# quoroom-ai/room

Measured on AMD Instinct MI355X. Metric: agent-cycles/sec, higher is better.
Workload: dtype bf16; 1 GPU; model=qwen3-coder-30b, agents_per_gpu=5, global_batch=5, seq_len=dynamic (session KV), parallelism=swarm-shard dp1 (one room shard/GPU, RCCL quorum)

## Files before the change

### room_amd/ops/csrc/flash_prefill.hip

```cpp
#include <torch/extension.h>
#include <c10/hip/HIPStream.h>
#include "common.h"
#include "kv_fp8.h"
#include "checks.h"

#define FP_BS 16
#define FP_QTOK 32
#define FP_CHUNK 64
#define FP_D 128
#define FP_QH 8
#define FP_PADK 8

typedef __attribute__((ext_vector_type(4))) float fpfrag_t;

template <bool F8>
__global__ __launch_bounds__(512, 1)
void flash_prefill_kernel(short* __restrict__ out,
                          const short* __restrict__ q,
                          const std::conditional_t<F8, uint8_t, short>*
                              __restrict__ kcache,
                          const std::conditional_t<F8, uint8_t, short>*
                              __restrict__ vcache,
                          const int* __restrict__ block_table,
                          const int* __restrict__ seq_ids,
                          const int* __restrict__ q_pos,
                          const int* __restrict__ tile_desc,
                          int n_kvheads, int max_blocks, int q_row_stride,
                          float scale,
                          const float* __restrict__ kscale,
                          const float* __restrict__ vscale) {
  const int g = blockIdx.x;
  const int hk = blockIdx.y;
  const int row0 = tile_desc[g * 2 + 0];
  const int ntok = tile_desc[g * 2 + 1];
  const int tid = threadIdx.x;
  const int wid = tid >> 6;
  const int lane = tid & 63;
  const int n_qheads = n_kvheads * FP_QH;
  const int hq = hk * FP_QH + wid;

  __shared__ short q_s[FP_QH][FP_QTOK][FP_D + FP_PADK];
  __shared__ short k_s[FP_CHUNK][FP_D + FP_PADK];
  __shared__ short vt_s[FP_D][FP_CHUNK + FP_PADK];
  __shared__ short p_s[FP_QH][FP_QTOK][FP_CHUNK + FP_PADK];
  __shared__ int qp_s[FP_QTOK];
  __shared__ int seq_s;

  #pragma unroll
  for (int it = 0; it < 8; ++it) {
    const int idx = tid + it * 512;
    const int h = idx / (FP_QTOK * FP_D / 8);
    const int rem = idx % (FP_QTOK * FP_D / 8);
    const int tk = rem / (FP_D / 8);
    const int d8 = (rem % (FP_D / 8)) * 8;
    bf16x8 v = {0, 0, 0, 0, 0, 0, 0, 0};
    if (tk < ntok) {
      v = *reinterpret_cast<const bf16x8*>(
          q + (long)(row0 + tk) * q_row_stride + (hk * FP_QH + h) * FP_D + d8);
      #pragma unroll
      for (int j = 0; j < 8; ++j) v[j] = f2bf(bf2f(v[j]) * scale);
    }
    *reinterpret_cast<bf16x8*>(&q_s[h][tk][d8]) = v;
  }
  if (tid < FP_QTOK)
    qp_s[tid] = (tid < ntok) ? q_pos[row0 + tid] : -1;
  if (tid == 0) seq_s = seq_ids[row0];
  __syncthreads();

  const int seq = seq_s;
  int bound_max = 0, bound_min = INT_MAX;
  for (int i = 0; i < ntok; ++i) {
    bound_max = max(bound_max, qp_s[i] + 1);
    bound_min = min(bound_min, qp_s[i] + 1);
  }
  const int* btab = block_table + (long)seq * max_blocks;
  const long kv_stride_block = (long)n_kvheads * FP_BS * FP_D;

  float m_run[2][4], l_run[2][4];
  fpfrag_t oacc[2][8];
  #pragma unroll
  for (int mt = 0; mt < 2; ++mt) {
    #pragma unroll
    for (int r = 0; r < 4; ++r) { m_run[mt][r] = -INFINITY; l_run[mt][r] = 0.f; }
    #pragma unroll
    for (int nf = 0; nf < 8; ++nf) oacc[mt][nf] = fpfrag_t{0.f, 0.f, 0.f, 0.f};
  }

  for (int base = 0; base < bound_max; base += FP_CHUNK) {
    #pragma unroll
    for (int it = 0; it < 2; ++it) {
      const int idx = tid + it * 512;
      const int pos_l = (idx * 8) / FP_D;
      const int d8 = (idx * 8) % FP_D;
      const int pos = base + pos_l;
      bf16x8 kv = {0, 0, 0, 0, 0, 0, 0, 0};
      bf16x8 vv = {0, 0, 0, 0, 0, 0, 0, 0};
      if (pos < bound_max) {
        const int blk = btab[pos / FP_BS];
        const long off = (long)blk * kv_stride_block
                         + ((long)hk * FP_BS + (pos % FP_BS)) * FP_D + d8;
        if constexpr (F8) {
          const long soff = ((long)blk * n_kvheads + hk) * FP_BS + pos % FP_BS;
          const kv_u32x2 kq = *reinterpret_cast<const kv_u32x2*>(kcache + off);
          const kv_u32x2 vq = *reinterpret_cast<const kv_u32x2*>(vcache + off);
          kv = __builtin_bit_cast(bf16x8, kv_fp8x8_to_bf16(kq, kscale[soff]));
          vv = __builtin_bit_cast(bf16x8, kv_fp8x8_to_bf16(vq, vscale[soff]));
        } else {
          kv = *reinterpret_cast<const bf16x8*>(kcache + off);
          vv = *reinterpret_cast<const bf16x8*>(vcache + off);
        }
      }
      *reinterpret_cast<bf16x8*>(&k_s[pos_l][d8]) = kv;
      #pragma unroll
      for (int j = 0; j < 8; ++j) vt_s[d8 + j][pos_l] = vv[j];
    }
    __syncthreads();

    fpfrag_t sfrag[2][4];
    #pragma unroll
    for (int mt = 0; mt < 2; ++mt)
      #pragma unroll
      for (int nt = 0; nt < 4; ++nt)
        sfrag[mt][nt] = fpfrag_t{0.f, 0.f, 0.f, 0.f};
    #pragma unroll
    for (int kk = 0; kk < 4; ++kk) {
      const int akoff = kk * 32 + (lane >> 4) * 8;
      bf16x8 a0 = *reinterpret_cast<const bf16x8*>(&q_s[wid][lane & 15][akoff]);
      bf16x8 a1 = *reinterpret_cast<const bf16x8*>(
          &q_s[wid][16 + (lane & 15)][akoff]);
      #pragma unroll
      for (int nt = 0; nt < 4; ++nt) {
        bf16x8 b = *reinterpret_cast<const bf16x8*>(
            &k_s[nt * 16 + (lane & 15)][akoff]);
        sfrag[0][nt] = __builtin_amdgcn_mfma_f32_16x16x32_bf16(a0, b, sfrag[0][nt], 0, 0, 0);
        sfrag[1][nt] = __builtin_amdgcn_mfma_f32_16x16x32_bf16(a1, b, sfrag[1][nt], 0, 0, 0);
      }
    }

    const int colL = lane & 15;
    const bool interior = (ntok == FP_QTOK) && (base + FP_CHUNK <= bound_min);
    #pragma unroll
    for (int mt = 0; mt < 2; ++mt) {
      #pragma unroll
      for (int r = 0; r < 4; ++r) {
        const int tk = mt * 16 + (lane >> 4) * 4 + r;
        const int bound = qp_s[tk] + 1;
        float sv[4];
        float mx = -INFINITY;
        if (interior) {
          #pragma unroll
          for (int nt = 0; nt < 4; ++nt) {
            sv[nt] = sfrag[mt][nt][r];
            mx = fmaxf(mx, sv[nt]);
          }
        } else {
          #pragma unroll
          for (int nt = 0; nt < 4; ++nt) {
            float s = sfrag[mt][nt][r];
            if (base + nt * 16 + colL >= bound) s = -INFINITY;
            sv[nt] = s;
            mx = fmaxf(mx, s);
          }
        }
        #pragma unroll
        for (int off = 8; off > 0; off >>= 1)
          mx = fmaxf(mx, __shfl_xor(mx, off, WAVE));
        const float m_new = fmaxf(m_run[mt][r], mx);
        float rs = 1.f, lsum = 0.f;
        float pv[4] = {0.f, 0.f, 0.f, 0.f};
        if (m_new != -INFINITY) {
          rs = (m_run[mt][r] == -INFINITY) ? 1.f : __expf(m_run[mt][r] - m_new);
          #pragma unroll
          for (int nt = 0; nt < 4; ++nt) {
            pv[nt] = (sv[nt] == -INFINITY) ? 0.f : __expf(sv[nt] - m_new);
            lsum += pv[nt];
          }
          #pragma unroll
          for (int off = 8; off > 0; off >>= 1)
            lsum += __shfl_xor(lsum, off, WAVE);
          l_run[mt][r] = l_run[mt][r] * rs + lsum;
          m_run[mt][r] = m_new;
        }
        #pragma unroll
        for (int nt = 0; nt < 4; ++nt)
          p_s[wid][tk][nt * 16 + colL] = f2bf(pv[nt]);
        if (rs != 1.f) {
          #pragma unroll
          for (int nf = 0; nf < 8; ++nf) oacc[mt][nf][r] *= rs;
        }
      }
    }
    __syncthreads();

    #pragma unroll
    for (int kk = 0; kk < 2; ++kk) {
      const int akoff = kk * 32 + (lane >> 4) * 8;
      bf16x8 a0 = *reinterpret_cast<const bf16x8*>(&p_s[wid][lane & 15][akoff]);
      bf16x8 a1 = *reinterpret_cast<const bf16x8*>(
          &p_s[wid][16 + (lane & 15)][akoff]);
      #pragma unroll
      for (int nf = 0; nf < 8; ++nf) {
        bf16x8 b = *reinterpret_cast<const bf16x8*>(
            &vt_s[nf * 16 + (lane & 15)][akoff]);
        oacc[0][nf] = __builtin_amdgcn_mfma_f32_16x16x32_bf16(a0, b, oacc[0][nf], 0, 0, 0);
        oacc[1][nf] = __builtin_amdgcn_mfma_f32_16x16x32_bf16(a1, b, oacc[1][nf], 0, 0, 0);
      }
    }
    __syncthreads();
  }

  #pragma unroll
  for (int mt = 0; mt < 2; ++mt) {
    #pragma unroll
    for (int r = 0; r < 4; ++r) {
      const int tk = mt * 16 + (lane >> 4) * 4 + r;
      if (tk >= ntok) continue;
      const float inv_l = (l_run[mt][r] > 0.f) ? 1.0f / l_run[mt][r] : 0.f;
      #pragma unroll
      for (int nf = 0; nf < 8; ++nf) {
        out[((long)(row0 + tk) * n_qheads + hq) * FP_D + nf * 16 + (lane & 15)] =
            f2bf(oacc[mt][nf][r] * inv_l);
      }
    }
  }
}

void flash_prefill(torch::Tensor out, torch::Tensor q, torch::Tensor kcache,
                   torch::Tensor vcache, torch::Tensor block_table,
                   torch::Tensor seq_ids, torch::Tensor q_pos,
                   torch::Tensor tile_desc, double scale,
                   c10::optional<torch::Tensor> k_scale,
                   c10::optional<torch::Tensor> v_scale) {
  OpChecks c("flash_prefill");
  const bool fp8 = kv_fp8_check(c, kcache, vcache, k_scale, v_scale);
  attn_check_tokens(c, out, q, kcache, block_table, seq_ids, q_pos);
  c.tensor("tile_desc", tile_desc, kI32, {-1, 2});
  const int n_kvheads = kcache.size(1);
  const int G = c.fits_int("tile_desc.size(0)", tile_desc.size(0));
  c.grid(G, n_kvheads);
  if (check_only()) return;
  const int max_blocks = block_table.size(1);
  dim3 grid(G, n_kvheads), block(512);
  hipStream_t s = c10::hip::getCurrentHIPStream();
  if (fp8)
    hipLaunchKernelGGL(flash_prefill_kernel<true>, grid, block, 0, s,
                       (short*)out.data_ptr(), (const short*)q.data_ptr(),
                       (const uint8_t*)kcache.data_ptr(),
                       (const uint8_t*)vcache.data_ptr(),
                       block_table.data_ptr<int>(), seq_ids.data_ptr<int>(),
                       q_pos.data_ptr<int>(), tile_desc.data_ptr<int>(),
                       n_kvheads, max_blocks, (int)q.stride(0), (float)scale,
                       k_scale->data_ptr<float>(), v_scale->data_ptr<float>());
  else
    hipLaunchKernelGGL(flash_prefill_kernel<false>, grid, block, 0, s,
                       (short*)out.data_ptr(), (const short*)q.data_ptr(),
                       (const short*)kcache.data_ptr(),
                       (const short*)vcache.data_ptr(),
                       block_table.data_ptr<int>(), seq_ids.data_ptr<int>(),
                       q_pos.data_ptr<int>(), tile_desc.data_ptr<int>(),
                       n_kvheads, max_blocks, (int)q.stride(0), (float)scale,
                       (const float*)nullptr, (const float*)nullptr);
  HIP_CHECK_KERNEL();
}

int64_t flash_prefill_qtile() { return FP_QTOK; }
```

Baseline: 6.390 cycles/s.

## Restructure flash prefill: register Q, double-buffered swizzled KV LDS, transposed V reads

Keeps Q fragments in registers instead of LDS and computes S transposed (K as the A operand), so the softmax probabilities stay in registers and feed the PV MFMA directly without a P round-trip through LDS. K/V tiles are double-buffered in XOR-swizzled LDS, and the next chunk's global loads are issued before the current chunk's compute, leaving one barrier per iteration. V is read with ds_read_tr16 transposed loads instead of a scalar transpose on store, and outputs are written packed. This adds register pressure and swizzle/transpose index complexity in exchange for less LDS traffic, fewer bank conflicts, fewer syncs and overlap of global loads with compute.

```diff
diff --git a/room_amd/ops/csrc/flash_prefill.hip b/room_amd/ops/csrc/flash_prefill.hip
--- a/room_amd/ops/csrc/flash_prefill.hip
+++ b/room_amd/ops/csrc/flash_prefill.hip
@@ -9,9 +9,17 @@
 #define FP_CHUNK 64
 #define FP_D 128
 #define FP_QH 8
-#define FP_PADK 8
+#define FP_TILE_B (FP_CHUNK * FP_D * 2)
 
 typedef __attribute__((ext_vector_type(4))) float fpfrag_t;
+typedef __attribute__((ext_vector_type(2))) float fp_f32x2;
+typedef __attribute__((ext_vector_type(2))) __bf16 fp_bf16x2;
+typedef __attribute__((address_space(3))) bf16x4 fp_lds_bf16x4;
+
+DEV uint32_t fp_pack_bf16(float lo, float hi) {
+  return __builtin_bit_cast(
+      uint32_t, __builtin_convertvector(fp_f32x2{lo, hi}, fp_bf16x2));
+}
 
 template <bool F8>
 __global__ __launch_bounds__(512, 1)
@@ -33,194 +41,237 @@
   const int hk = blockIdx.y;
   const int row0 = tile_desc[g * 2 + 0];
   const int ntok = tile_desc[g * 2 + 1];
+  if (ntok <= 0) return;
   const int tid = threadIdx.x;
   const int wid = tid >> 6;
   const int lane = tid & 63;
+  const int lrow = lane & 15;
+  const int lgrp = lane >> 4;
   const int n_qheads = n_kvheads * FP_QH;
   const int hq = hk * FP_QH + wid;
 
-  __shared__ short q_s[FP_QH][FP_QTOK][FP_D + FP_PADK];
-  __shared__ short k_s[FP_CHUNK][FP_D + FP_PADK];
-  __shared__ short vt_s[FP_D][FP_CHUNK + FP_PADK];
-  __shared__ short p_s[FP_QH][FP_QTOK][FP_CHUNK + FP_PADK];
-  __shared__ int qp_s[FP_QTOK];
-  __shared__ int seq_s;
-
-  #pragma unroll
-  for (int it = 0; it < 8; ++it) {
-    const int idx = tid + it * 512;
-    const int h = idx / (FP_QTOK * FP_D / 8);
-    const int rem = idx % (FP_QTOK * FP_D / 8);
-    const int tk = rem / (FP_D / 8);
-    const int d8 = (rem % (FP_D / 8)) * 8;
-    bf16x8 v = {0, 0, 0, 0, 0, 0, 0, 0};
+  __shared__ __attribute__((aligned(16))) char kv_s[2][2][FP_TILE_B];
+
+  bf16x8 qf[2][4];
+  int bnd[2];
+  #pragma unroll
+  for (int mt = 0; mt < 2; ++mt) {
+    const int tk = mt * 16 + lrow;
+    bnd[mt] = 0;
+    #pragma unroll
+    for (int kk = 0; kk < 4; ++kk) qf[mt][kk] = bf16x8{0, 0, 0, 0, 0, 0, 0, 0};
     if (tk < ntok) {
-      v = *reinterpret_cast<const bf16x8*>(
-          q + (long)(row0 + tk) * q_row_stride + (hk * FP_QH + h) * FP_D + d8);
-      #pragma unroll
-      for (int j = 0; j < 8; ++j) v[j] = f2bf(bf2f(v[j]) * scale);
-    }
-    *reinterpret_cast<bf16x8*>(&q_s[h][tk][d8]) = v;
+      bnd[mt] = q_pos[row0 + tk] + 1;
+      const short* qp = q + (long)(row0 + tk) * q_row_stride + hq * FP_D
+                        + lgrp * 8;
+      #pragma unroll
+      for (int kk = 0; kk < 4; ++kk) {
+        bf16x8 v = *reinterpret_cast<const bf16x8*>(qp + kk * 32);
+        #pragma unroll
+        for (int j = 0; j < 8; ++j) v[j] = f2bf(bf2f(v[j]) * scale);
+        qf[mt][kk] = v;
+      }
+    }
   }
-  if (tid < FP_QTOK)
-    qp_s[tid] = (tid < ntok) ? q_pos[row0 + tid] : -1;
-  if (tid == 0) seq_s = seq_ids[row0];
-  __syncthreads();
-
-  const int seq = seq_s;
-  int bound_max = 0, bound_min = INT_MAX;
-  for (int i = 0; i < ntok; ++i) {
-    bound_max = max(bound_max, qp_s[i] + 1);
-    bound_min = min(bound_min, qp_s[i] + 1);
+  int bmax = max(bnd[0], bnd[1]), bmin = min(bnd[0], bnd[1]);
+  #pragma unroll
+  for (int off = 8; off > 0; off >>= 1) {
+    bmax = max(bmax, __shfl_xor(bmax, off, WAVE));
+    bmin = min(bmin, __shfl_xor(bmin, off, WAVE));
   }
+  const int bound_max = __builtin_amdgcn_readfirstlane(bmax);
+  const int bound_min = __builtin_amdgcn_readfirstlane(bmin);
+
+  const int seq = seq_ids[row0];
   const int* btab = block_table + (long)seq * max_blocks;
   const long kv_stride_block = (long)n_kvheads * FP_BS * FP_D;
 
-  float m_run[2][4], l_run[2][4];
+  using raw_t = std::conditional_t<F8, kv_u32x2, bf16x8>;
+  const int srow = tid >> 4, sch = tid & 15;
+  const long slice_off = ((long)hk * FP_BS + (srow & 15)) * FP_D + sch * 8;
+  const int k_wr = srow * 256 + ((sch ^ (srow & 15)) << 4);
+  const int v_wr = srow * 256 + ((sch ^ ((srow & 7) << 1)) << 4);
+  raw_t kraw[2], vraw[2];
+  float ksc[2], vsc[2];
+  int blk[2];
+
+  auto load_blk = [&](int base) {
+    #pragma unroll
+    for (int it = 0; it < 2; ++it) {
+      const int pos = base + srow + it * 32;
+      blk[it] = (pos < bound_max) ? btab[pos / FP_BS] : 0;
+    }
+  };
+  auto issue = [&](int base) {
+    #pragma unroll
+    for (int it = 0; it < 2; ++it) {
+      const int pos = base + srow + it * 32;
+      kraw[it] = raw_t{};
+      vraw[it] = raw_t{};
+      ksc[it] = vsc[it] = 1.f;
+      if (pos < bound_max) {
+        const long off = (long)blk[it] * kv_stride_block + slice_off;
+        kraw[it] = *reinterpret_cast<const raw_t*>(kcache + off);
+        vraw[it] = *reinterpret_cast<const raw_t*>(vcache + off);
+        if constexpr (F8) {
+          const long soff = ((long)blk[it] * n_kvheads + hk) * FP_BS
+                            + (srow & 15);
+          ksc[it] = kscale[soff];
+          vsc[it] = vscale[soff];
+        }
+      }
+    }
+  };
+  auto commit = [&](int b) {
+    #pragma unroll
+    for (int it = 0; it < 2; ++it) {
+      bf16x8 kv, vv;
+      if constexpr (F8) {
+        kv = __builtin_bit_cast(bf16x8, kv_fp8x8_to_bf16(kraw[it], ksc[it]));
+        vv = __builtin_bit_cast(bf16x8, kv_fp8x8_to_bf16(vraw[it], vsc[it]));
+      } else {
+        kv = kraw[it];
+        vv = vraw[it];
+      }
+      *reinterpret_cast<bf16x8*>(&kv_s[b][0][k_wr + it * 32 * 256]) = kv;
+      *reinterpret_cast<bf16x8*>(&kv_s[b][1][v_wr + it * 32 * 256]) = vv;
+    }
+  };
+
+  int k_rd[4];
+  #pragma unroll
+  for (int kk = 0; kk < 4; ++kk)
+    k_rd[kk] = lrow * 256 + (((kk * 4 + lgrp) ^ lrow) << 4);
+  const int v_q = lrow >> 2, v_p = lrow & 3;
+  const int v_x = 4 * (lgrp & 1) + v_q;
+  const int v_rd = (4 * lgrp + v_q) * 256 + v_p * 8;
+
+  float m_run[2] = {-INFINITY, -INFINITY};
+  float l_run[2] = {0.f, 0.f};
   fpfrag_t oacc[2][8];
   #pragma unroll
-  for (int mt = 0; mt < 2; ++mt) {
-    #pragma unroll
-    for (int r = 0; r < 4; ++r) { m_run[mt][r] = -INFINITY; l_run[mt][r] = 0.f; }
+  for (int mt = 0; mt < 2; ++mt)
     #pragma unroll
     for (int nf = 0; nf < 8; ++nf) oacc[mt][nf] = fpfrag_t{0.f, 0.f, 0.f, 0.f};
-  }
-
-  for (int base = 0; base < bound_max; base += FP_CHUNK) {
-    #pragma unroll
-    for (int it = 0; it < 2; ++it) {
-      const int idx = tid + it * 512;
-      const int pos_l = (idx * 8) / FP_D;
-      const int d8 = (idx * 8) % FP_D;
-      const int pos = base + pos_l;
-      bf16x8 kv = {0, 0, 0, 0, 0, 0, 0, 0};
-      bf16x8 vv = {0, 0, 0, 0, 0, 0, 0, 0};
-      if (pos < bound_max) {
-        const int blk = btab[pos / FP_BS];
-        const long off = (long)blk * kv_stride_block
-                         + ((long)hk * FP_BS + (pos % FP_BS)) * FP_D + d8;
-        if constexpr (F8) {
-          const long soff = ((long)blk * n_kvheads + hk) * FP_BS + pos % FP_BS;
-          const kv_u32x2 kq = *reinterpret_cast<const kv_u32x2*>(kcache + off);
-          const kv_u32x2 vq = *reinterpret_cast<const kv_u32x2*>(vcache + off);
-          kv = __builtin_bit_cast(bf16x8, kv_fp8x8_to_bf16(kq, kscale[soff]));
-          vv = __builtin_bit_cast(bf16x8, kv_fp8x8_to_bf16(vq, vscale[soff]));
-        } else {
-          kv = *reinterpret_cast<const bf16x8*>(kcache + off);
-          vv = *reinterpret_cast<const bf16x8*>(vcache + off);
+
+  load_blk(0);
+  issue(0);
+  load_blk(FP_CHUNK);
+  commit(0);
+  __syncthreads();
+
+  int cur = 0;
+  for (int base = 0; base < bound_max; base += FP_CHUNK, cur ^= 1) {
+    const bool more = base + FP_CHUNK < bound_max;
+    if (more) {
+      issue(base + FP_CHUNK);
+      load_blk(base + 2 * FP_CHUNK);
+    }
+    const char* kb = kv_s[cur][0];
+    const char* vb = kv_s[cur][1];
+
+    fpfrag_t st[2][4];
+    #pragma unroll
+    for (int mt = 0; mt < 2; ++mt)
+      #pragma unroll
+      for (int nt = 0; nt < 4; ++nt)
+        st[mt][nt] = fpfrag_t{0.f, 0.f, 0.f, 0.f};
+    #pragma unroll
+    for (int kk = 0; kk < 4; ++kk) {
+      #pragma unroll
+      for (int nt = 0; nt < 4; ++nt) {
+        const bf16x8 a = *reinterpret_cast<const bf16x8*>(
+            kb + nt * 16 * 256 + k_rd[kk]);
+        st[0][nt] = __builtin_amdgcn_mfma_f32_16x16x32_bf16(a, qf[0][kk], st[0][nt], 0, 0, 0);
+        st[1][nt] = __builtin_amdgcn_mfma_f32_16x16x32_bf16(a, qf[1][kk], st[1][nt], 0, 0, 0);
+      }
+    }
+
+    const bool interior = (ntok == FP_QTOK) && (base + FP_CHUNK <= bound_min);
+    float rs[2];
+    bf16x8 pb[2][2];
+    #pragma unroll
+    for (int mt = 0; mt < 2; ++mt) {
+      if (!interior) {
+        const int lim = bnd[mt] - base - 4 * lgrp;
+        #pragma unroll
+        for (int nt = 0; nt < 4; ++nt)
+          #pragma unroll
+          for (int r = 0; r < 4; ++r)
+            if (nt * 16 + r >= lim) st[mt][nt][r] = -INFINITY;
+      }
+      float mx = -INFINITY;
+      #pragma unroll
+      for (int nt = 0; nt < 4; ++nt)
+        #pragma unroll
+        for (int r = 0; r < 4; ++r) mx = fmaxf(mx, st[mt][nt][r]);
+      mx = fmaxf(mx, __shfl_xor(mx, 16, WAVE));
+      mx = fmaxf(mx, __shfl_xor(mx, 32, WAVE));
+      const float m_new = fmaxf(m_run[mt], mx);
+      const float m_safe = (m_new == -INFINITY) ? 0.f : m_new;
+      rs[mt] = (m_run[mt] == m_new) ? 1.f : __expf(m_run[mt] - m_safe);
+      float psum = 0.f;
+      #pragma unroll
+      for (int nt = 0; nt < 4; ++nt)
+        #pragma unroll
+        for (int r = 0; r < 4; ++r) {
+          const float p = __expf(st[mt][nt][r] - m_safe);
+          st[mt][nt][r] = p;
+          psum += p;
         }
-      }
-      *reinterpret_cast<bf16x8*>(&k_s[pos_l][d8]) = kv;
-      #pragma unroll
-      for (int j = 0; j < 8; ++j) vt_s[d8 + j][pos_l] = vv[j];
-    }
-    __syncthreads();
-
-    fpfrag_t sfrag[2][4];
-    #pragma unroll
-    for (int mt = 0; mt < 2; ++mt)
-      #pragma unroll
-      for (int nt = 0; nt < 4; ++nt)
-        sfrag[mt][nt] = fpfrag_t{0.f, 0.f, 0.f, 0.f};
-    #pragma unroll
-    for (int kk = 0; kk < 4; ++kk) {
-      const int akoff = kk * 32 + (lane >> 4) * 8;
-      bf16x8 a0 = *reinterpret_cast<const bf16x8*>(&q_s[wid][lane & 15][akoff]);
-      bf16x8 a1 = *reinterpret_cast<const bf16x8*>(
-          &q_s[wid][16 + (lane & 15)][akoff]);
-      #pragma unroll
-      for (int nt = 0; nt < 4; ++nt) {
-        bf16x8 b = *reinterpret_cast<const bf16x8*>(
-            &k_s[nt * 16 + (lane & 15)][akoff]);
-        sfrag[0][nt] = __builtin_amdgcn_mfma_f32_16x16x32_bf16(a0, b, sfrag[0][nt], 0, 0, 0);
-        sfrag[1][nt] = __builtin_amdgcn_mfma_f32_16x16x32_bf16(a1, b, sfrag[1][nt], 0, 0, 0);
-      }
-    }
-
-    const int colL = lane & 15;
-    const bool interior = (ntok == FP_QTOK) && (base + FP_CHUNK <= bound_min);
-    #pragma unroll
-    for (int mt = 0; mt < 2; ++mt) {
-      #pragma unroll
-      for (int r = 0; r < 4; ++r) {
-        const int tk = mt * 16 + (lane >> 4) * 4 + r;
-        const int bound = qp_s[tk] + 1;
-        float sv[4];
-        float mx = -INFINITY;
-        if (interior) {
-          #pragma unroll
-          for (int nt = 0; nt < 4; ++nt) {
-            sv[nt] = sfrag[mt][nt][r];
-            mx = fmaxf(mx, sv[nt]);
-          }
-        } else {
-          #pragma unroll
-          for (int nt = 0; nt < 4; ++nt) {
-            float s = sfrag[mt][nt][r];
-            if (base + nt * 16 + colL >= bound) s = -INFINITY;
-            sv[nt] = s;
-            mx = fmaxf(mx, s);
-          }
-        }
-        #pragma unroll
-        for (int off = 8; off > 0; off >>= 1)
-          mx = fmaxf(mx, __shfl_xor(mx, off, WAVE));
-        const float m_new = fmaxf(m_run[mt][r], mx);
-        float rs = 1.f, lsum = 0.f;
-        float pv[4] = {0.f, 0.f, 0.f, 0.f};
-        if (m_new != -INFINITY) {
-          rs = (m_run[mt][r] == -INFINITY) ? 1.f : __expf(m_run[mt][r] - m_new);
-          #pragma unroll
-          for (int nt = 0; nt < 4; ++nt) {
-            pv[nt] = (sv[nt] == -INFINITY) ? 0.f : __expf(sv[nt] - m_new);
-            lsum += pv[nt];
-          }
-          #pragma unroll
-          for (int off = 8; off > 0; off >>= 1)
-            lsum += __shfl_xor(lsum, off, WAVE);
-          l_run[mt][r] = l_run[mt][r] * rs + lsum;
-          m_run[mt][r] = m_new;
-        }
-        #pragma unroll
-        for (int nt = 0; nt < 4; ++nt)
-          p_s[wid][tk][nt * 16 + colL] = f2bf(pv[nt]);
-        if (rs != 1.f) {
-          #pragma unroll
-          for (int nf = 0; nf < 8; ++nf) oacc[mt][nf][r] *= rs;
-        }
-      }
-    }
-    __syncthreads();
-
-    #pragma unroll
-    for (int kk = 0; kk < 2; ++kk) {
-      const int akoff = kk * 32 + (lane >> 4) * 8;
-      bf16x8 a0 = *reinterpret_cast<const bf16x8*>(&p_s[wid][lane & 15][akoff]);
-      bf16x8 a1 = *reinterpret_cast<const bf16x8*>(
-          &p_s[wid][16 + (lane & 15)][akoff]);
+      l_run[mt] = l_run[mt] * rs[mt] + psum;
+      m_run[mt] = m_new;
+      #pragma unroll
+      for (int s = 0; s < 2; ++s) {
+        const kv_u32x4 w = {
+            fp_pack_bf16(st[mt][2 * s][0], st[mt][2 * s][1]),
+            fp_pack_bf16(st[mt][2 * s][2], st[mt][2 * s][3]),
+            fp_pack_bf16(st[mt][2 * s + 1][0], st[mt][2 * s + 1][1]),
+            fp_pack_bf16(st[mt][2 * s + 1][2], st[mt][2 * s + 1][3])};
+        pb[mt][s] = __builtin_bit_cast(bf16x8, w);
+      }
+    }
+    if (!__all(rs[0] == 1.f && rs[1] == 1.f)) {
+      #pragma unroll
+      for (int mt = 0; mt < 2; ++mt)
+        #pragma unroll
+        for (int nf = 0; nf < 8; ++nf) oacc[mt][nf] *= rs[mt];
+    }
+
+    #pragma unroll
+    for (int s = 0; s < 2; ++s) {
       #pragma unroll
       for (int nf = 0; nf < 8; ++nf) {
-        bf16x8 b = *reinterpret_cast<const bf16x8*>(
-            &vt_s[nf * 16 + (lane & 15)][akoff]);
-        oacc[0][nf] = __builtin_amdgcn_mfma_f32_16x16x32_bf16(a0, b, oacc[0][nf], 0, 0, 0);
-        oacc[1][nf] = __builtin_amdgcn_mfma_f32_16x16x32_bf16(a1, b, oacc[1][nf], 0, 0, 0);
-      }
-    }
+        const char* va = vb + s * 32 * 256 + v_rd + (((2 * nf) ^ (v_x << 1)) << 4);
+        const bf16x4 lo = __builtin_amdgcn_ds_read_tr16_b64_v4i16(
+            (fp_lds_bf16x4*)(va));
+        const bf16x4 hi = __builtin_amdgcn_ds_read_tr16_b64_v4i16(
+            (fp_lds_bf16x4*)(va + 16 * 256));
+        const bf16x8 a = {lo[0], lo[1], lo[2], lo[3], hi[0], hi[1], hi[2], hi[3]};
+        oacc[0][nf] = __builtin_amdgcn_mfma_f32_16x16x32_bf16(a, pb[0][s], oacc[0][nf], 0, 0, 0);
+        oacc[1][nf] = __builtin_amdgcn_mfma_f32_16x16x32_bf16(a, pb[1][s], oacc[1][nf], 0, 0, 0);
+      }
+    }
+
+    if (more) commit(cur ^ 1);
     __syncthreads();
   }
 
   #pragma unroll
   for (int mt = 0; mt < 2; ++mt) {
-    #pragma unroll
-    for (int r = 0; r < 4; ++r) {
-      const int tk = mt * 16 + (lane >> 4) * 4 + r;
-      if (tk >= ntok) continue;
-      const float inv_l = (l_run[mt][r] > 0.f) ? 1.0f / l_run[mt][r] : 0.f;
-      #pragma unroll
-      for (int nf = 0; nf < 8; ++nf) {
-        out[((long)(row0 + tk) * n_qheads + hq) * FP_D + nf * 16 + (lane & 15)] =
-            f2bf(oacc[mt][nf][r] * inv_l);
-      }
+    float l = l_run[mt];
+    l += __shfl_xor(l, 16, WAVE);
+    l += __shfl_xor(l, 32, WAVE);
+    const float inv_l = (l > 0.f) ? 1.0f / l : 0.f;
+    const int tk = mt * 16 + lrow;
+    if (tk >= ntok) continue;
+    short* orow = out + ((long)(row0 + tk) * n_qheads + hq) * FP_D + 4 * lgrp;
+    #pragma unroll
+    for (int nf = 0; nf < 8; ++nf) {
+      const kv_u32x2 w = {
+          fp_pack_bf16(oacc[mt][nf][0] * inv_l, oacc[mt][nf][1] * inv_l),
+          fp_pack_bf16(oacc[mt][nf][2] * inv_l, oacc[mt][nf][3] * inv_l)};
+      *reinterpret_cast<kv_u32x2*>(orow + nf * 16) = w;
     }
   }
 }
```

New measurement: 7.033 cycles/s, median of 6. +10.1%, better.
